# imazen/codec-eval

Hardware: AMD Instinct MI355X
Metric: metric MP/s (SSIMULACRA2+DSSIM+Butteraugli) at 1/2/4/8 GPU; HBM-roofline % (higher is better)
Workload: dtype f32

## Files before the change

codec-eval_amd/csrc/butteraugli.hip:

```cpp
#include <algorithm>
#include <cmath>
#include <cstdlib>
#include <type_traits>

#include "ce_internal.h"

namespace {

constexpr int TPB = 256;
constexpr int PSY = 10;
enum { UHF0 = 0, UHF1, HF0, HF1, MF0, MF1, MF2, LF0, LF1, LF2 };

struct geom {
    uint32_t w, h, pitch;
    size_t plane;
};

struct blur_kernel {
    int len;
    float k[40];
    float lo[16], hi[16];
};

#define BA_XY                                                           \
// ... 370 lines not shown
    constexpr int NF = (RAW * (IW / 4) + TPB - 1) / TPB;
    float4 pf[NF];
    auto fetch = [&](int q) {
        const float *p = tmp + (EPI == EPI_MASK ? (size_t)slot : (size_t)slot * 3 + q) * g.plane;
#pragma unroll
        for (int m = 0; m < NF; m++) {
            const int i = m * TPB + (int)threadIdx.x, r = i / (IW / 4), X = x0 - (HV ? LEFT : 0) + 4 * (i % (IW / 4)), Y = y0 - off + r;
            float4 v = make_float4(0.f, 0.f, 0.f, 0.f);
            if (r < RAW && Y >= 0 && Y < (int)g.h && X >= 0 && X < (int)g.pitch) v = *reinterpret_cast<const float4 *>(p + (size_t)Y * g.pitch + X);
            v.x = X < (int)g.w ? v.x : 0.0f;
            v.y = X + 1 < (int)g.w ? v.y : 0.0f;
            v.z = X + 2 < (int)g.w ? v.z : 0.0f;
            v.w = X + 3 < (int)g.w ? v.w : 0.0f;
            pf[m] = v;
        }
    };
    auto stash = [&]() {
#pragma unroll
        for (int m = 0; m < NF; m++) {
            const int i = m * TPB + (int)threadIdx.x;
            if (i < RAW * (IW / 4)) *reinterpret_cast<float4 *>((HV ? in_t : tile) + 4 * i) = pf[m];
        }
    };
    constexpr int S0 = LEFT - off, NW = (S0 + 3 + LEN + 3) / 4;
    const int rc4 = 4 * ((int)threadIdx.x % (TW / 4));
    __shared__ __attribute__((aligned(16))) float s_sx[HV ? TW : 4];
    if (HV && threadIdx.x < TW)
        s_sx[threadIdx.x] = x0 + (int)threadIdx.x < (int)g.w ? border_scale<LEN>(bk, x0 + (int)threadIdx.x, (int)g.w, inv_wsum) : 0.0f;
    float scale_x[4] = {0.0f, 0.0f, 0.0f, 0.0f};
    fetch(0);
    if (HV) {
        stash();
        __syncthreads();
#pragma unroll
        for (int k = 0; k < 4; k++) scale_x[k] = s_sx[rc4 + k];
    }
#pragma unroll
    for (int q = 0; q < NP; q++) {
        if (HV) {
#pragma unroll 1
            for (int u = threadIdx.x; u < RAW * (TW / 4); u += TPB) {
                const int r = u / (TW / 4);
                const float4 *src = reinterpret_cast<const float4 *>(in_t + r * IW + rc4);
                float wnd[4 * NW];
#pragma unroll
                for (int m = 0; m < NW; m++) {
                    const float4 v = src[m];
                    wnd[4 * m] = v.x, wnd[4 * m + 1] = v.y, wnd[4 * m + 2] = v.z, wnd[4 * m + 3] = v.w;
                }
                float out[4];
#pragma unroll
                for (int k = 0; k < 4; k++) {
                    float sum = 0.0f;
#pragma unroll
                    for (int j = 0; j < LEN; j++) sum = blur_tap(sum, wnd[S0 + k + j], bk.k[j]);
                    out[k] = sum * scale_x[k];
                }
                *reinterpret_cast<float4 *>(tile + r * TW + rc4) = make_float4(out[0], out[1], out[2], out[3]);
            }
            __syncthreads();
            if (q + 1 < NP) fetch(q + 1);
        } else {
            if (q) __syncthreads();
            stash();
            if (q + 1 < NP) fetch(q + 1);
            __syncthreads();
        }
#pragma unroll
        for (int part = 0; part < PARTS; part++) {
            const int ly = 32 * part + 8 * wv, gy0 = y0 + ly;
            if (col_live && gy0 < (int)g.h) {
                float v[BW_OUT + LEN - 1];
#pragma unroll
                for (int j = 0; j < BW_OUT + LEN - 1; j++) v[j] = tile[(ly + j) * TW + c];
#pragma unroll
                for (int o = 0; o < BW_OUT; o++) {
                    float sum = 0.0f;
#pragma unroll
                    for (int j = 0; j < LEN; j++) sum = blur_tap(sum, v[o + j], bk.k[j]);
                    res[q][part][o] = sum * border_scale<LEN>(bk, gy0 + o, (int)g.h, inv_wsum);
                }
            }
        }
        if (HV && q + 1 < NP) {
            stash();
            __syncthreads();
        }
    }
    if (!col_live) return;
    const size_t pl = g.plane;
#pragma unroll
    for (int part = 0; part < PARTS; part++) {
        const int gy0 = y0 + 32 * part + 8 * wv;
        if (gy0 >= (int)g.h) break;
        float *ps = psy + (size_t)slot * PSY * g.plane + (size_t)gy0 * g.pitch + gx;
#pragma unroll
        for (int o = 0; o < BW_OUT; o++) {
            if (gy0 + o >= (int)g.h) break;
            float *q = ps + (size_t)o * g.pitch;
            const size_t ao = (size_t)slot * 3 * pl + (size_t)(gy0 + o) * g.pitch + gx;
            if (EPI == EPI_LF) {
                const float *xs = xyb + (size_t)slot * 3 * pl + (size_t)(gy0 + o) * g.pitch + gx;
                const float lx = res[0][part][o], ly = res[1][part][o], lb = res[2][part][o];
                aux_out[ao] = xs[0] - lx;
                aux_out[ao + pl] = xs[pl] - ly;
                aux_out[ao + 2 * pl] = xs[2 * pl] - lb;
                const float xmul = 33.832837186260f, ymul = 14.458268100570f, bmul = 49.87984651440f, y_to_b_mul = -0.362267051518f;
                const float bb = __builtin_fmaf(y_to_b_mul, ly, lb);
                q[LF2 * pl] = bb * bmul;
                q[LF0 * pl] = lx * xmul;
                q[LF1 * pl] = ly * ymul;
            } else if (EPI == EPI_MF) {
                const float kRemoveMfRange = 0.29f, kAddMfRange = 0.1f;
                const float mf0 = res[0][part][o], mf1 = res[1][part][o];
                const float hf0 = tmp[ao] - mf0, hf1 = tmp[ao + pl] - mf1;
                q[MF0 * pl] = remove_range(kRemoveMfRange, mf0);
                q[MF1 * pl] = amplify_range(kAddMfRange, mf1);
                q[MF2 * pl] = res[2][part][o];
                const float suppress = 46.0f, sv = 0.653020556257f, one_minus_s = 1.0f - 0.653020556257f;
                const float scaler = __builtin_fmaf(suppress / __builtin_fmaf(hf1, hf1, suppress), one_minus_s, sv);
                aux_out[ao] = scaler * hf0;
                aux_out[ao + pl] = hf1;
            } else if (EPI == EPI_MASK) {
                aux_out[(size_t)slot * pl + (size_t)(gy0 + o) * g.pitch + gx] = res[0][part][o];
            } else {
                const float kRemoveHfRange = 1.5f, kAddHfRange = 0.132f, kRemoveUhfRange = 0.04f;
                const float kMaxclampHf = 28.4691806922f, kMaxclampUhf = 5.19175294647f, kMulYHf = 2.155f, kMulYUhf = 2.69313763794f;
                float hf0_out, uhf0_out, hf1_out, uhf1_out;
                {
                    const float hf = res[0][part][o];
                    const float uhf = tmp[ao] - hf;
                    hf0_out = remove_range(kRemoveHfRange, hf);
                    uhf0_out = remove_range(kRemoveUhfRange, uhf);
                    q[HF0 * pl] = hf0_out;
                    q[UHF0 * pl] = uhf0_out;
                }
                {
                    float hf = maximum_clamp(res[1][part][o], kMaxclampHf);
                    float uhf = tmp[ao + pl] - hf;
                    uhf = maximum_clamp(uhf, kMaxclampUhf);
                    uhf *= kMulYUhf;
                    uhf1_out = uhf;
                    q[UHF1 * pl] = uhf;
                    hf *= kMulYHf;
                    hf1_out = amplify_range(kAddHfRange, hf);
                    q[HF1 * pl] = hf1_out;
                }
                mask_in[(size_t)slot * pl + (size_t)(gy0 + o) * g.pitch + gx] = mask_pre_one(uhf0_out, hf0_out, uhf1_out, hf1_out);
            }
        }
    }
}

struct malta_params {
    float norm2_0gt1, norm2_0lt1, norm1;
};

struct mline {
    int n;
    signed char d[9][2];
};

__device__ constexpr mline MALTA_HF[16] = {
    {9, {{-4, 0}, {-3, 0}, {-2, 0}, {-1, 0}, {0, 0}, {1, 0}, {2, 0}, {3, 0}, {4, 0}}},
    {9, {{0, -4}, {0, -3}, {0, -2}, {0, -1}, {0, 0}, {0, 1}, {0, 2}, {0, 3}, {0, 4}}},
    {7, {{-3, -3}, {-2, -2}, {-1, -1}, {0, 0}, {1, 1}, {2, 2}, {3, 3}}},
    {7, {{3, -3}, {2, -2}, {1, -1}, {0, 0}, {-1, 1}, {-2, 2}, {-3, 3}}},
    {9, {{1, -4}, {1, -3}, {1, -2}, {0, -1}, {0, 0}, {0, 1}, {-1, 2}, {-1, 3}, {-1, 4}}},
    {9, {{-1, -4}, {-1, -3}, {-1, -2}, {0, -1}, {0, 0}, {0, 1}, {1, 2}, {1, 3}, {1, 4}}},
    {9, {{-4, -1}, {-3, -1}, {-2, -1}, {-1, 0}, {0, 0}, {1, 0}, {2, 1}, {3, 1}, {4, 1}}},
    {9, {{-4, 1}, {-3, 1}, {-2, 1}, {-1, 0}, {0, 0}, {1, 0}, {2, -1}, {3, -1}, {4, -1}}},
    {7, {{-2, -3}, {-1, -2}, {-1, -1}, {0, 0}, {1, 1}, {1, 2}, {2, 3}}},
    {7, {{2, -3}, {1, -2}, {1, -1}, {0, 0}, {-1, 1}, {-1, 2}, {-2, 3}}},
    {7, {{-3, -2}, {-2, -1}, {-1, -1}, {0, 0}, {1, 1}, {2, 1}, {3, 2}}},
    {7, {{3, -2}, {2, -1}, {1, -1}, {0, 0}, {-1, 1}, {-2, 1}, {-3, 2}}},
    {8, {{-4, 2}, {-3, 2}, {-2, 1}, {-1, 1}, {0, 0}, {1, 0}, {2, -1}, {3, -1}}},
    {8, {{-4, -2}, {-3, -2}, {-2, -1}, {-1, -1}, {0, 0}, {1, 0}, {2, 1}, {3, 1}}},
    {8, {{-2, -4}, {-2, -3}, {-1, -2}, {-1, -1}, {0, 0}, {0, 1}, {1, 2}, {1, 3}}},
    {8, {{2, -4}, {2, -3}, {1, -2}, {1, -1}, {0, 0}, {0, 1}, {-1, 2}, {-1, 3}}},
};
__device__ constexpr mline MALTA_LF[16] = {
    {5, {{-4, 0}, {-2, 0}, {0, 0}, {2, 0}, {4, 0}}},
    {5, {{0, -4}, {0, -2}, {0, 0}, {0, 2}, {0, 4}}},
    {5, {{-3, -3}, {-2, -2}, {0, 0}, {2, 2}, {3, 3}}},
    {5, {{3, -3}, {2, -2}, {0, 0}, {-2, 2}, {-3, 3}}},
    {5, {{1, -4}, {1, -2}, {0, 0}, {-1, 2}, {-1, 4}}},
    {5, {{-1, -4}, {-1, -2}, {0, 0}, {1, 2}, {1, 4}}},
    {5, {{-4, -1}, {-2, -1}, {0, 0}, {2, 1}, {4, 1}}},
    {5, {{-4, 1}, {-2, 1}, {0, 0}, {2, -1}, {4, -1}}},
    {5, {{-2, -3}, {-1, -2}, {0, 0}, {1, 2}, {2, 3}}},
    {5, {{2, -3}, {1, -2}, {0, 0}, {-1, 2}, {-2, 3}}},
    {5, {{-3, -2}, {-2, -1}, {0, 0}, {2, 1}, {3, 2}}},
    {5, {{3, -2}, {2, -1}, {0, 0}, {-2, 1}, {-3, 2}}},
    {5, {{-4, 2}, {-2, 1}, {0, 0}, {2, -1}, {4, -2}}},
    {5, {{-4, -2}, {-2, -1}, {0, 0}, {2, 1}, {4, 2}}},
    {5, {{-2, -4}, {-1, -2}, {0, 0}, {1, 2}, {2, 4}}},
    {5, {{2, -4}, {1, -2}, {0, 0}, {-1, 2}, {-2, 4}}},
};

constexpr int MT = 64, MH = 4, ML = MT + 2 * MH;

__device__ constexpr bool malta_line_descends(const mline &ln)
{
    for (int j = 1; j < ln.n; j++)
        if (ln.d[j][1] > ln.d[j - 1][1]) return false;
    return ln.d[0][1] != ln.d[ln.n - 1][1];
}
__device__ constexpr bool malta_line_monotone(const mline &ln)
{
    bool up = true, down = true;
    for (int j = 1; j < ln.n; j++) {
        if (ln.d[j][1] < ln.d[j - 1][1]) up = false;
        if (ln.d[j][1] > ln.d[j - 1][1]) down = false;
    }
    return up || down;
}
__device__ constexpr bool malta_tables_monotone()
{
    for (int k = 0; k < 16; k++)
        if (!malta_line_monotone(MALTA_HF[k]) || !malta_line_monotone(MALTA_LF[k])) return false;
    return true;
}
static_assert(malta_tables_monotone(), "the row-streaming Malta unit needs every line's rows to be visited in one direction");

struct malta_bands {
    malta_params p[2][3];
};

__device__ __forceinline__ void div2_shared_rcp(float a0, float a1, float b, float &q0, float &q1)
{
    const float r = ce_rcp_refined(b);
    q0 = ce_div_refined(a0, b, r);
    q1 = ce_div_refined(a1, b, r);
}

__device__ __forceinline__ float malta_pre_diff(float v0, float v1, const malta_params &mp)
{
    const float absval = 0.5f * (fabsf(v0) + fabsf(v1));
    const float diff = v0 - v1;
    float scaler, scaler2;
    div2_shared_rcp(mp.norm2_0gt1, mp.norm2_0lt1, mp.norm1 + absval, scaler, scaler2);
    const float r = scaler * diff;
    const float fabs0 = fabsf(v0), too_small = 0.55f * fabs0, too_big = 1.05f * fabs0;
    const bool neg = v0 < 0;
    const float u = neg ? -v1 : v1;
    const bool lo = u < too_small, hi = u > too_big;
    const float impact = scaler2 * (lo ? too_small - u : u - too_big);
    const float rn = r + ((neg == lo) ? -impact : impact);
    return (lo || hi) ? rn : r;
}

__device__ __forceinline__ float l2_asym_acc(float total, float val0, float val1, float vw_0gt1, float vw_0lt1)
{
    const float diff = val0 - val1;
    total = __builtin_fmaf(diff * diff, vw_0gt1, total);
    const float fabs0 = fabsf(val0);
    const float too_small = 0.4f * fabs0, too_big = fabs0;
    const float if_neg = val1 > -too_small ? val1 + too_small : (val1 < -too_big ? -val1 - too_big : 0.0f);
    const float if_pos = val1 < too_small ? too_small - val1 : (val1 > too_big ? val1 - too_big : 0.0f);
    const float v = val0 < 0.0f ? if_neg : if_pos;
    return __builtin_fmaf(vw_0lt1, v * v, total);
}

template <bool LF>
__device__ __forceinline__ void malta_rows_xy(const ba_f2 *__restrict__ base, ba_f2 (&acc)[2])
{
    ba_f2 sum[2][16];
    ba_f2 parked[2][16][9];
#pragma unroll
    for (int r = 0; r < 9; r++) {
        ba_f2 v[10];
        const float4 *row = reinterpret_cast<const float4 *>(base + r * ML);
#pragma unroll
        for (int q = 0; q < 5; q++) {
            const float4 t = row[q];
            v[2 * q] = ba_f2{t.x, t.y};
            v[2 * q + 1] = ba_f2{t.z, t.w};
        }
        const int dy = r - 4;
#pragma unroll
        for (int o = 0; o < 2; o++) {
#pragma unroll
            for (int k = 0; k < 16; k++) {
                const mline &ln = LF ? MALTA_LF[k] : MALTA_HF[k];
                if (!malta_line_descends(ln)) {
#pragma unroll
                    for (int j = 0; j < 9; j++)
                        if (j < ln.n && ln.d[j][1] == dy) {
                            const ba_f2 t = v[4 + o + ln.d[j][0]];
                            sum[o][k] = j == 0 ? t : sum[o][k] + t;
                        }
                } else if (dy == ln.d[0][1]) {
                    ba_f2 acc_k = {0.0f, 0.0f};
#pragma unroll
                    for (int j = 0; j < 9; j++)
                        if (j < ln.n) {
                            const ba_f2 t = ln.d[j][1] == dy ? v[4 + o + ln.d[j][0]] : parked[o][k][j];
                            acc_k = j == 0 ? t : acc_k + t;
                        }
                    sum[o][k] = acc_k;
                } else {
#pragma unroll
                    for (int j = 0; j < 9; j++)
                        if (j < ln.n && ln.d[j][1] == dy) parked[o][k][j] = v[4 + o + ln.d[j][0]];
                }
            }
// ... 366 lines not shown
        b->ba_psy[l] = b->ba_diff[l] = b->ba_mask[l] = nullptr;
    }
    for (auto &p : b->ba_s) hipFree(p), p = nullptr;
    for (auto &p : b->ba_s_half) hipFree(p), p = nullptr;
    if (b->ba_half_stream) hipStreamSynchronize(b->ba_half_stream);
    if (b->ev_ba_fork) hipEventDestroy(b->ev_ba_fork);
    if (b->ev_ba_join) hipEventDestroy(b->ev_ba_join);
    b->ba_half_stream = nullptr;
    b->ev_ba_fork = b->ev_ba_join = nullptr;
    hipFree(b->ba_blk_max);
    hipFree(b->ba_blk_sums);
    hipFree(b->ba_pnorm);
    hipFree(b->ba_map);
    hipFree(b->ba_cells);
    b->ba_map = b->ba_cells = nullptr;
    b->ba_cells_cap = 0;
    b->ba_map_pairs = 0;
    b->ba_blk_max = nullptr;
    b->ba_blk_sums = nullptr;
    b->ba_pnorm = nullptr;
    b->ba_ref_src = nullptr;
    b->ba_ready = false;
}

static int ba_allocate(ce_batch *b)
{
    ce_ctx *ctx = b->ctx;
    auto set = [](ce_batch::ba_level &d, uint32_t w, uint32_t h) {
        d.w = w;
        d.h = h;
        d.pitch = (w + 31u) & ~31u;
        d.plane = (size_t)d.pitch * h;
    };
    set(b->ba[0], b->w, b->h);
    set(b->ba[1], (b->w + 1) / 2, (b->h + 1) / 2);
    b->ba_levels = (b->ba[1].w >= 8 && b->ba[1].h >= 8) ? 2 : 1;
    const size_t slots = (size_t)b->max_refs + b->max_pairs, P = b->max_pairs, p0 = b->ba[0].plane;
    for (int l = 0; l < b->ba_levels; l++) {
        CE_HIP(ctx, hipMalloc(&b->ba_psy[l], slots * PSY * b->ba[l].plane * sizeof(float)));
        if (l == 1) CE_HIP(ctx, hipMalloc(&b->ba_diff[l], P * b->ba[l].plane * sizeof(float)));
    }
    for (auto &p : b->ba_s) CE_HIP(ctx, hipMalloc(&p, slots * 3 * p0 * sizeof(float)));
    for (int l = 0; l < b->ba_levels; l++) {
        CE_HIP(ctx, hipMalloc(&b->ba_mask[l], slots * b->ba[l].plane * sizeof(float)));
        CE_HIP(ctx, hipMalloc(&b->ba_mask_vals[l], (size_t)b->max_refs * 2 * b->ba[l].plane * sizeof(float)));
    }
    b->ba_blocks = ((b->ba[0].w + 63) / 64) * ((b->ba[0].h + 3) / 4);
    CE_HIP(ctx, hipMalloc(&b->ba_blk_max, P * b->ba_blocks * sizeof(float)));
    CE_HIP(ctx, hipMalloc(&b->ba_blk_sums, P * b->ba_blocks * 3 * sizeof(double)));
    CE_HIP(ctx, hipMalloc(&b->ba_pnorm, P * sizeof(double)));
    return CE_OK;
}

static int ba_prepare(ce_batch *b)
{
    if (b->ba_ready) return CE_OK;
    const int rc = ba_allocate(b);
    if (rc != CE_OK) {
        const std::string why = b->ctx->err;
        ce_butteraugli_free(b);
        (void)hipGetLastError();
        b->ctx->err = why;
        return rc;
    }
    b->ba_ready = true;
    return CE_OK;
}

int ce_launch_butteraugli(ce_batch *b, const uint8_t *d_refs, uint32_t n_refs_used, uint32_t n_pairs, float intensity_target,
                          bool store_map)
{
    ce_ctx *ctx = b->ctx;
    int rc = ba_prepare(b);
    if (rc != CE_OK) return rc;
    if (store_map && !b->ba_map && hipMalloc(&b->ba_map, (size_t)b->max_pairs * b->ba[0].plane * sizeof(float)) != hipSuccess) {
        b->ba_map = nullptr;
        (void)hipGetLastError();
        ctx->err = "out of device memory for the Butteraugli diffmaps";
        return CE_ERR_BACKEND;
    }
    const uint32_t n_slots = n_refs_used + n_pairs, mr = b->max_refs;
    const bool cached = b->keep_ref_pyramid && b->ba_ref_src == d_refs && b->ba_ref_count >= n_refs_used && b->ba_ref_intensity == intensity_target;
    const uint32_t z0 = cached ? n_refs_used : 0, nz = n_slots - z0;
    if (!cached) b->ref_builds[2]++;
    const blur_kernel k12 = make_kernel(1.2f), kLf = make_kernel(7.15593339443f), kHf = make_kernel(3.22489901262f),
                      kUhf = make_kernel(1.56416327805f), kMask = make_kernel(2.7f);
    float sw = 0.0f;
    for (int j = 0; j < 5; j++) sw += k12.k[j];
    const float sc = 1.0f / sw, w0 = k12.k[2] * sc, w1 = k12.k[3] * sc, w2 = k12.k[4] * sc;
    const double hf_asymmetry = 1.0;
    const malta_params mUhfY = make_malta(1.10039032555 * hf_asymmetry, 1.10039032555 / hf_asymmetry, 71.7800275169, false);
    const malta_params mUhfX = make_malta(173.5 * hf_asymmetry, 173.5 / hf_asymmetry, 5.0, false);
    const malta_params mHfY = make_malta(18.7237414387 * std::sqrt(hf_asymmetry), 18.7237414387 / std::sqrt(hf_asymmetry), 4498534.45232, true);
    const malta_params mHfX = make_malta(6923.99476109 * std::sqrt(hf_asymmetry), 6923.99476109 / std::sqrt(hf_asymmetry), 8051.15833247, true);
    const malta_params mMfY = make_malta(37.0819870399, 37.0819870399, 130262059.556, true);
    const malta_params mMfX = make_malta(8246.75321353, 8246.75321353, 1009002.70582, true);

    const bool two_streams = b->ba_levels == 2 && !ctx->prof_serial && (double)n_pairs * b->w * b->h <= 4e6;
    hipStream_t s_main = CE_STREAM(ctx), s_half = s_main;
    if (two_streams) {
        if (!b->ba_half_stream) {
            if (!(b->ba_half_stream = ce_ctx_aux_stream(ctx, ce_ctx::AUX_BA_HALF))) return CE_ERR_BACKEND;
            CE_HIP(ctx, hipEventCreateWithFlags(&b->ev_ba_fork, hipEventDisableTiming));
            CE_HIP(ctx, hipEventCreateWithFlags(&b->ev_ba_join, hipEventDisableTiming));
            const size_t slots = (size_t)b->max_refs + b->max_pairs;
            for (auto &p : b->ba_s_half) CE_HIP(ctx, hipMalloc(&p, slots * 3 * b->ba[1].plane * sizeof(float)));
        }
        s_half = b->ba_half_stream;
        CE_HIP(ctx, hipEventRecord(b->ev_ba_fork, s_main));
        CE_HIP(ctx, hipStreamWaitEvent(s_half, b->ev_ba_fork, 0));
    }
    uint32_t final_tiles = 0;
    for (int l = b->ba_levels - 1; l >= 0; l--) {
        const auto &d = b->ba[l];
        const geom g{d.w, d.h, d.pitch, d.plane};
        const dim3 gx((d.w + 63) / 64, (d.h + 3) / 4, 1);
        auto G = [&](uint32_t z) { return dim3(gx.x, gx.y, z); };
        hipStream_t st = l == 1 ? s_half : s_main;
        float *const *scr = (two_streams && l == 1) ? b->ba_s_half : b->ba_s;
        float *psy = b->ba_psy[l], *sA = scr[0], *sC = scr[2];
        const plane_sel s3{3, 0, 3};
        const dim3 ft((d.w + FT - 1) / FT, (d.h + FT - 1) / FT, nz);
        if (l == 0) {
            CE_LAUNCH_ON(ctx, st, "ba_front_u8", k_ba_front<false>, ft, dim3(TPB), 0, d_refs, b->d_tests, ctx->d_lut_ssim2, g, sC, g, w0, w1, w2,
                      intensity_target, b->img_bytes, n_refs_used, mr, z0);
        } else {
            const auto &pd = b->ba[0];
            CE_LAUNCH_ON(ctx, st, "ba_front_half", k_ba_front<true>, ft, dim3(TPB), 0, d_refs, b->d_tests, ctx->d_lut_ssim2,
                      geom{pd.w, pd.h, pd.pitch, pd.plane}, sC, g, w0, w1, w2, intensity_target, b->img_bytes, n_refs_used, mr, z0);
        }
        {
            if (kLf.len != 33 || kHf.len != 15 || kUhf.len != 7) {
                ctx->err = "unexpected blur kernel length";
                return CE_ERR_BACKEND;
            }
            const dim3 gh3((g.w + 255) / 256, (g.h + 8 * BH_TILES - 1) / (8 * BH_TILES), nz * 3);
            float *sB = scr[1];
            CE_LAUNCH_ON(ctx, st, "ba_blur_h33", k_ba_blur_h<33>, gh3, dim3(TPB), 0, (const float *)sC, sA, g, s3, s3, kLf, inv_weight_sum(kLf),
                      n_refs_used, mr, 1, z0);
            const dim3 gvs((g.w + 63) / 64, (g.h + 31) / 32, nz);
            CE_LAUNCH_ON(ctx, st, "ba_blur_v_lf", (k_ba_blur_v_split<33, EPI_LF, false, 32>), gvs, dim3(TPB), 0, (const float *)sA,
                         (const float *)sC, psy, g, kLf, inv_weight_sum(kLf), n_refs_used, mr, z0, (float *)nullptr, sB);
            CE_LAUNCH_ON(ctx, st, "ba_blur_hv_mf", (k_ba_blur_v_split<15, EPI_MF, true, 32>), gvs, dim3(TPB), 0, (const float *)sB,
                         (const float *)nullptr, psy, g, kHf, inv_weight_sum(kHf), n_refs_used, mr, z0, (float *)nullptr, sA);
            CE_LAUNCH_ON(ctx, st, "ba_blur_hv_hf", (k_ba_blur_v_split<7, EPI_HF, true, 32>), gvs, dim3(TPB), 0, (const float *)sA,
                         (const float *)nullptr, psy, g, kUhf, inv_weight_sum(kUhf), n_refs_used, mr, z0, sB, (float *)nullptr);
        }

        {
            if (kMask.len != 13) {
                ctx->err = "unexpected blur kernel length";
                return CE_ERR_BACKEND;
            }
            const dim3 gm((g.w + 63) / 64, (g.h + 31) / 32, nz);
            CE_LAUNCH_ON(ctx, st, "ba_blur_hv_mask", (k_ba_blur_v_split<13, EPI_MASK, true, 32>), gm, dim3(TPB), 0, (const float *)scr[1],
                      (const float *)nullptr, psy, g, kMask, inv_weight_sum(kMask), n_refs_used, mr, z0, (float *)nullptr, b->ba_mask[l]);
        }
        if (!cached)
            CE_LAUNCH_ON(ctx, st, "ba_mask_vals", k_ba_mask_vals, G(n_refs_used), dim3(TPB), 0, (const float *)b->ba_mask[l], b->ba_mask_vals[l], g);

        malta_bands mb;
        mb.p[0][0] = mUhfX; mb.p[0][1] = mHfX; mb.p[0][2] = mMfX;
        mb.p[1][0] = mUhfY; mb.p[1][1] = mHfY; mb.p[1][2] = mMfY;
        const uint32_t tiles_x = (d.w + MT - 1) / MT, tiles_y = (d.h + 31) / 32;
        if ((rc = ce_build_xcd_list(b, n_pairs, ce_xcd_keys{1, tiles_x * tiles_y, 1}, &b->ba_work[l])) != CE_OK) return rc;
        const bool has_sub = b->ba_levels == 2;
        const auto &ds = b->ba[has_sub ? 1 : 0];
        const geom gsub{ds.w, ds.h, ds.pitch, ds.plane};
#define CE_MALTA_ARGS(FINAL, STORE)                                                                                                \
    psy, b->d_pair_ref, (const float *)b->ba_mask[l], (const float *)b->ba_mask_vals[l],                                               \
        STORE ? b->ba_map : FINAL ? (float *)nullptr : b->ba_diff[1], g, mr, mb, (const uint2 *)b->ba_work[l].d, tiles_x,             \
        FINAL ? (const float *)b->ba_diff[1] : (const float *)nullptr, gsub, has_sub ? 1 : 0, b->ba_blk_max, b->ba_blk_sums, b->ba_blocks
        const dim3 gmalta(b->ba_work[l].len);
        if (l == 0) {
            final_tiles = tiles_x * tiles_y;
            if (two_streams) CE_HIP(ctx, hipStreamWaitEvent(s_main, b->ev_ba_join, 0));
            if (store_map)
                CE_LAUNCH_ON(ctx, st, "ba_malta_l2_map", (k_ba_malta_l2_xy<32, 256, true, true>), gmalta, dim3(256), 0, CE_MALTA_ARGS(true, true));
            else
                CE_LAUNCH_ON(ctx, st, "ba_malta_l2", (k_ba_malta_l2_xy<32, 256, true, false>), gmalta, dim3(256), 0, CE_MALTA_ARGS(true, false));
        } else {
            CE_LAUNCH_ON(ctx, st, "ba_malta_l2", (k_ba_malta_l2_xy<32, 256, false, false>), gmalta, dim3(256), 0, CE_MALTA_ARGS(false, false));
            if (two_streams) CE_HIP(ctx, hipEventRecord(b->ev_ba_join, s_half));
        }
#undef CE_MALTA_ARGS
    }
    if (b->keep_ref_pyramid && !cached) {
        b->ba_ref_src = d_refs;
        b->ba_ref_count = n_refs_used;
        b->ba_ref_intensity = intensity_target;
    }
    const auto &d0 = b->ba[0];
    CE_LAUNCH(ctx, "ba_score", k_ba_score, dim3(n_pairs), dim3(TPB), 0, b->ba_blk_max, b->ba_blk_sums, b->d_scores, b->ba_pnorm,
              b->ba_blocks, final_tiles, (double)d0.w * (double)d0.h);
    CE_HIP(ctx, hipGetLastError());
    return CE_OK;
}

int ce_butteraugli_read_maps(ce_batch *b, uint32_t first, uint32_t count, uint32_t block, float *out)
{
    ce_ctx *ctx = b->ctx;
    const auto &d = b->ba[0];
    const geom g{d.w, d.h, d.pitch, d.plane};
    if (block == 1) {
        CE_HIP(ctx, hipMemcpy2DAsync(out, (size_t)d.w * sizeof(float), b->ba_map + (size_t)first * d.plane, (size_t)d.pitch * sizeof(float),
                                     (size_t)d.w * sizeof(float), (size_t)count * d.h, hipMemcpyDeviceToHost, ctx->stream));
        CE_HIP(ctx, hipStreamSynchronize(ctx->stream));
        return CE_OK;
    }
    uint32_t lb = 0;
    while ((1u << lb) < block) lb++;
    const uint32_t bw = (d.w + block - 1) >> lb, bh = (d.h + block - 1) >> lb, tiles_x = (d.w + 255) / 256;
    const size_t n = (size_t)count * bw * bh;
    if (b->ba_cells_cap < n) {
        hipFree(b->ba_cells);
        b->ba_cells = nullptr;
        b->ba_cells_cap = 0;
        CE_HIP(ctx, hipMalloc(&b->ba_cells, n * sizeof(float)));
        b->ba_cells_cap = n;
    }
    const size_t blocks = (size_t)tiles_x * bh * count;
    if (blocks > 0x7fffffffu) {
        ctx->err = "diffmap readout too large for one launch";
        return CE_ERR_INVALID_ARG;
    }
    CE_LAUNCH_ON(ctx, ctx->stream, "ba_block_max", k_ba_block_max, dim3((uint32_t)blocks), dim3(256), 0, (const float *)b->ba_map, g, first,
                 lb, tiles_x, bw, bh, b->ba_cells);
    CE_HIP(ctx, hipGetLastError());
    CE_HIP(ctx, hipMemcpyAsync(out, b->ba_cells, n * sizeof(float), hipMemcpyDeviceToHost, ctx->stream));
    CE_HIP(ctx, hipStreamSynchronize(ctx->stream));
    return CE_OK;
}
```

profiles/make_traffic.py:

```python
#!/usr/bin/env python3
import collections
import csv
import glob
import importlib
import json
import os
import re
import sys

HERE = os.path.dirname(os.path.abspath(__file__))
sys.path.insert(0, os.path.dirname(HERE))

SHORT = [
    (r"k_ssim2_hblur_lds<-1>", "ssim2_hblur_L1-5"), (r"k_ssim2_vblur_dma<-1>", "ssim2_vblur_ssim_L1-5"),
    (r"k_ssim2_hblur_lds<0>", "ssim2_hblur_L0"), (r"k_ssim2_vblur_dma<0>", "ssim2_vblur_ssim_L0"),
    (r"k_ssim2_prep<true>", "ssim2_prep_u8"), (r"k_ssim2_prep<false>", "ssim2_prep"), (r"k_ssim2_finalize", "ssim2_finalize"),
    (r"k_dssim_create_stream<true", "dssim_create_u8"), (r"k_dssim_create_stream<false", "dssim_create"), (r"k_dssim_create<true>", "dssim_create_u8"), (r"k_dssim_create<false>", "dssim_create"), (r"k_dssim_compare", "dssim_compare"),
    (r"k_dssim_avg", "dssim_avg"), (r"k_dssim_absdev", "dssim_absdev"), (r"k_dssim_finalize_pairs", "dssim_finalize"),
    (r"k_ba_front<false>", "ba_front_u8"), (r"k_ba_front<true>", "ba_front_half"), (r"k_ba_subsample2x_u8", "ba_subsample2x"),
    (r"k_ba_blur_h<(\d+)>", "ba_blur_h{}"), (r"k_ba_blur_v<(\d+)>", "ba_blur_v{}"),
    (r"k_ba_blur_v_split<13", "ba_blur_hv_mask"), (r"k_ba_blur_v_split<33", "ba_blur_v_lf"), (r"k_ba_blur_v_split<15, *1, *true", "ba_blur_hv_mf"), (r"k_ba_blur_v_split<7, *2, *true", "ba_blur_hv_hf"),
    (r"k_ba_blur_v_split<15", "ba_blur_v_mf"), (r"k_ba_blur_v_split<7", "ba_blur_v_hf"),
    (r"k_ba_malta_l2_xy", "ba_malta_l2"), (r"k_ba_mask_pre", "ba_mask_pre"), (r"k_ba_mask_vals", "ba_mask_vals"), (r"k_ba_mask_combine", "ba_mask_combine"),
    (r"k_ba_final", "ba_final"), (r"k_ba_score", "ba_score"), (r"k_psnr_sse", "psnr_sse"), (r"k_psnr_clear", "psnr_clear"),
    (r"k_xyb_roundtrip", "xyb_roundtrip"), (r"k_calib_read<(\d+)>", "calib_read_b{}"), (r"k_calib_write<(\d+)>", "calib_write_b{}"),
]
READ_WIDTH_16 = ("ssim2_hblur", "ssim2_vblur", "ba_blur_h", "ba_blur_v_", "ba_malta_l2")
READ_WIDTH_1 = ("dssim_create_u8", "ba_subsample2x")
WRITE_WIDTH_16 = ("ssim2_hblur", "ba_blur_h")


def short(name):
    for pat, fmt in SHORT:
        m = re.search(pat, name)
        if m:
            return fmt.format(*m.groups())
    return name.split("(")[0][-48:]


def one(d, suffix):
    f = glob.glob(os.path.join(d, "**", "*" + suffix), recursive=True)
    if not f:
        raise SystemExit(f"no *{suffix} under {d}")
    return max(f, key=os.path.getmtime)


def counters_of(d, cname):
    acc, n = collections.defaultdict(float), collections.Counter()
    for r in csv.DictReader(open(one(d, "counter_collection.csv"))):
        if r["Counter_Name"] != cname:
            continue
        k = short(r["Kernel_Name"])
        acc[k] += float(r["Counter_Value"])
        n[k] += 1
    return {k: acc[k] / n[k] for k in acc}, dict(n)


def main():
    if sys.argv[1] == "--stats-only":
        tag, fetch_dir, write_dir, sidecar = None, None, None, None
        stats_dir, stats_tag = sys.argv[2], sys.argv[3]
    else:
        tag, fetch_dir, write_dir, sidecar = sys.argv[1:5]
        stats_dir = sys.argv[5] if len(sys.argv) > 5 else None
        stats_tag = sys.argv[6] if len(sys.argv) > 6 else tag
    if stats_dir:
        rows = list(csv.DictReader(open(one(stats_dir, "kernel_stats.csv"))))
        with open(os.path.join(HERE, f"{stats_tag}_kernel_stats.csv"), "w", newline="") as fo:
            w = csv.writer(fo)
            w.writerow(["Kernel", "Calls", "TotalDurationNs", "AverageNs", "Percentage", "MinNs", "MaxNs"])
            groups = collections.OrderedDict()
            for r in rows:
                groups.setdefault(short(r["Name"]), []).append(r)
            for name, rs in groups.items():
                if len(rs) == 1:
                    r = rs[0]
                    w.writerow([name, r["Calls"], r["TotalDurationNs"], r["AverageNs"], r["Percentage"], r["MinNs"], r["MaxNs"]])
                    continue
                calls = sum(int(r["Calls"]) for r in rs)
                total = sum(int(r["TotalDurationNs"]) for r in rs)
                w.writerow([name, calls, total, f"{total / calls:.6f}", f"{sum(float(r['Percentage']) for r in rs):.2f}",
                            min(int(r["MinNs"]) for r in rs), max(int(r["MaxNs"]) for r in rs)])
                for r in rs:
                    inst = re.search(r"<([^>]*)>", r["Name"])
                    w.writerow([f"{name} [instance <{inst.group(1) if inst else '?'}>]", r["Calls"], r["TotalDurationNs"], r["AverageNs"],
                                r["Percentage"], r["MinNs"], r["MaxNs"]])
    if sidecar is None:
        return
    side = json.load(open(sidecar))
    rf = importlib.import_module("codec-eval_amd.roofline")
    alg = rf.step_bytes([rf.Bucket(side["width"], side["height"], side["n_refs"], side["n_pairs"])], side["metrics"], side["xyb_roundtrip"])
    px0 = side["n_pairs"] * side["width"] * side["height"]
    fetch, n_f = counters_of(fetch_dir, "FETCH_SIZE")
    write, n_w = counters_of(write_dir, "WRITE_SIZE")
    cal = side["calib_bytes"]
    f_read = {w_: cal / (fetch[f"calib_read_b{w_}"] * 1024) for w_ in (1, 4, 16) if fetch.get(f"calib_read_b{w_}")}
    f_write = {w_: cal / (write[f"calib_write_b{w_}"] * 1024) for w_ in (4, 16) if write.get(f"calib_write_b{w_}")}
    out = {
        "_provenance": "rocprofv3 --kernel-trace --pmc FETCH_SIZE / --pmc WRITE_SIZE, two separate passes over "
                       f"profiles/prof_step.py {side['config']} {side['steps']}; counters are KiB, averaged per launch; corrected by the "
                       "per-width factors MEASURED in the same passes from the calibration streams (bytes moved / bytes reported); "
                       "produced by profiles/make_traffic.py",
        "_launch": dict(side, scale0_pixels=px0),
        "_calibration": {"read_factor_by_lane_bytes": {str(k): round(v, 4) for k, v in f_read.items()},
                         "write_factor_by_lane_bytes": {str(k): round(v, 4) for k, v in f_write.items()}},
    }
    with open(os.path.join(HERE, f"{tag}_pmc_fetch_write.csv"), "w", newline="") as fo:
        w = csv.writer(fo)
        w.writerow(["Kernel", "launches_per_step", "FETCH_SIZE_KiB_per_launch", "WRITE_SIZE_KiB_per_launch"])
        for k in sorted(set(fetch) | set(write)):
            f, wr = fetch.get(k, 0.0), write.get(k, 0.0)
            lps = n_f.get(k, n_w.get(k, 0)) / (1 if k.startswith("calib_") else side["steps"])
            w.writerow([k, round(lps, 2), round(f, 1), round(wr, 1)])
            if k.startswith(("calib_", "__amd")):
                continue
            rw = 16 if k.startswith(READ_WIDTH_16) else 1 if k.startswith(READ_WIDTH_1) else 4
            ww = 16 if k.startswith(WRITE_WIDTH_16) else 4
            fb = f * 1024 * f_read.get(rw, 1.0)
            wb = wr * 1024 * f_write.get(ww, 1.0)
            per_step = (fb + wb) * lps
            out[k] = {"launches_per_step": round(lps, 2), "fetch_bytes_per_launch": fb, "write_bytes_per_launch": wb,
                      "hbm_bytes_per_launch": fb + wb, "hbm_bytes_per_step": per_step, "bytes_per_scale0_pixel": round(per_step / px0, 2),
                      "read_lane_bytes": rw, "write_lane_bytes": ww}
            if k in alg:
                out[k]["algorithmic_bytes_per_step"] = alg[k]
                out[k]["algorithmic_bytes_per_scale0_pixel"] = round(alg[k] / px0, 2)
                out[k]["traffic_over_algorithmic"] = round(per_step / alg[k], 3)
    json.dump(out, open(os.path.join(HERE, f"traffic_{tag}.json"), "w"), indent=1)
    print("calibration", out["_calibration"])
    for k, v in out.items():
        if not k.startswith("_"):
            print(f"{k:24s} {v['bytes_per_scale0_pixel']:8.2f} B/px0   alg {v.get('algorithmic_bytes_per_scale0_pixel', float('nan')):8.2f}")


if __name__ == "__main__":
    main()
```

Measured before the change: 19040.

## Replace mask blur with single-wave vertical strip kernel using register sliding window

Adds a new separable blur kernel for the mask stage. Each 64-thread block walks down a 64-column strip: it prefetches rows into registers, runs the horizontal pass through LDS, and keeps the vertical window in registers, so halo rows are not re-read per tile. Strip height is picked adaptively to keep enough waves in flight. The trade-off is more serial work per block and fewer threads per block, which can hurt occupancy and latency hiding on small images.

```diff
diff --git a/codec-eval_amd/csrc/butteraugli.hip b/codec-eval_amd/csrc/butteraugli.hip
--- a/codec-eval_amd/csrc/butteraugli.hip
+++ b/codec-eval_amd/csrc/butteraugli.hip
@@ -546,6 +546,103 @@
     }
 }
 
+template <int LEN>
+__global__ __launch_bounds__(64) void k_ba_blur_hv_strip(const float *__restrict__ in, float *__restrict__ out, geom g, blur_kernel bk,
+                                                         float inv_wsum, uint32_t n_refs_used, uint32_t max_refs, uint32_t z0, uint32_t sh)
+{
+    constexpr int off = LEN / 2, TW = 64, SR = 8, LEFT = 8, IW = TW + 2 * LEFT;
+    static_assert(off <= LEFT, "row-pass halo");
+    constexpr int P = (LEN - 1 + SR - 1) / SR, PAD = P * SR - (LEN - 1), WN = (P + 1) * SR;
+    __shared__ __attribute__((aligned(16))) float in_t[SR * IW];
+    __shared__ __attribute__((aligned(16))) float rb[SR * TW];
+    __shared__ __attribute__((aligned(16))) float s_sx[TW];
+    const uint32_t slot = slot_of(blockIdx.z + z0, n_refs_used, max_refs);
+    const float *p = in + (size_t)slot * g.plane;
+    const int x0 = blockIdx.x * TW, ys = blockIdx.y * (int)sh, ye = min(ys + (int)sh, (int)g.h);
+    const int t = threadIdx.x, gx = x0 + t;
+    const int y_in = ys - off - PAD, steps = P + (ye - ys + SR - 1) / SR;
+    constexpr int NF = (SR * (IW / 4) + 63) / 64;
+    float4 pf[NF];
+    auto fetch = [&](int y) {
+#pragma unroll
+        for (int m = 0; m < NF; m++) {
+            const int i = m * 64 + t, r = i / (IW / 4), X = x0 - LEFT + 4 * (i % (IW / 4)), Y = y + r;
+            float4 v = make_float4(0.f, 0.f, 0.f, 0.f);
+            if (r < SR && Y >= 0 && Y < (int)g.h && X >= 0 && X < (int)g.pitch) v = *reinterpret_cast<const float4 *>(p + (size_t)Y * g.pitch + X);
+            v.x = X < (int)g.w ? v.x : 0.0f;
+            v.y = X + 1 < (int)g.w ? v.y : 0.0f;
+            v.z = X + 2 < (int)g.w ? v.z : 0.0f;
+            v.w = X + 3 < (int)g.w ? v.w : 0.0f;
+            pf[m] = v;
+        }
+    };
+    constexpr int S0 = LEFT - off, NW = (S0 + 3 + LEN + 3) / 4;
+    const int rc4 = 4 * (t % (TW / 4)), rr = t / (TW / 4);
+    s_sx[t] = gx < (int)g.w ? border_scale<LEN>(bk, gx, (int)g.w, inv_wsum) : 0.0f;
+    fetch(y_in);
+    __syncthreads();
+    float scale_x[4];
+#pragma unroll
+    for (int k = 0; k < 4; k++) scale_x[k] = s_sx[rc4 + k];
+    float win[WN];
+#pragma unroll
+    for (int j = 0; j < WN; j++) win[j] = 0.0f;
+#pragma unroll 1
+    for (int s = 0; s < steps; s++) {
+#pragma unroll
+        for (int m = 0; m < NF; m++) {
+            const int i = m * 64 + t;
+            if (i < SR * (IW / 4)) *reinterpret_cast<float4 *>(in_t + 4 * i) = pf[m];
+        }
+        if (s + 1 < steps) fetch(y_in + SR * (s + 1));
+        __syncthreads();
+#pragma unroll
+        for (int h2 = 0; h2 < SR / 4; h2++) {
+            const int r = rr + 4 * h2;
+            const float4 *src = reinterpret_cast<const float4 *>(in_t + r * IW + rc4);
+            float wnd[4 * NW];
+#pragma unroll
+            for (int m = 0; m < NW; m++) {
+                const float4 v = src[m];
+                wnd[4 * m] = v.x, wnd[4 * m + 1] = v.y, wnd[4 * m + 2] = v.z, wnd[4 * m + 3] = v.w;
+            }
+            float o4[4];
+#pragma unroll
+            for (int k = 0; k < 4; k++) {
+                float sum = 0.0f;
+#pragma unroll
+                for (int j = 0; j < LEN; j++) sum = blur_tap(sum, wnd[S0 + k + j], bk.k[j]);
+                o4[k] = sum * scale_x[k];
+            }
+            *reinterpret_cast<float4 *>(rb + r * TW + rc4) = make_float4(o4[0], o4[1], o4[2], o4[3]);
+        }
+        __syncthreads();
+#pragma unroll
+        for (int j = 0; j < WN - SR; j++) win[j] = win[j + SR];
+#pragma unroll
+        for (int r = 0; r < SR; r++) win[WN - SR + r] = rb[r * TW + t];
+        if (s < P || gx >= (int)g.w) continue;
+        const int y0 = ys + SR * (s - P);
+#pragma unroll
+        for (int o = 0; o < SR; o++) {
+            if (y0 + o >= ye) break;
+            float sum = 0.0f;
+#pragma unroll
+            for (int j = 0; j < LEN; j++) sum = blur_tap(sum, win[PAD + o + j], bk.k[j]);
+            out[(size_t)slot * g.plane + (size_t)(y0 + o) * g.pitch + gx] = sum * border_scale<LEN>(bk, y0 + o, (int)g.h, inv_wsum);
+        }
+    }
+}
+
+uint32_t ba_strip_rows(uint32_t strips, uint32_t h, uint32_t n_images)
+{
+    auto waves = [&](uint32_t rows) { return (size_t)strips * ((h + rows - 1) / rows) * n_images; };
+    uint32_t rows = 128;
+    while (rows > 32 && waves(rows) < 8192) rows /= 2;
+    while (rows > 8 && waves(rows) < 2048) rows /= 2;
+    return rows;
+}
+
 struct malta_params {
     float norm2_0gt1, norm2_0lt1, norm1;
 };
@@ -1218,9 +1315,9 @@
                 ctx->err = "unexpected blur kernel length";
                 return CE_ERR_BACKEND;
             }
-            const dim3 gm((g.w + 63) / 64, (g.h + 31) / 32, nz);
-            CE_LAUNCH_ON(ctx, st, "ba_blur_hv_mask", (k_ba_blur_v_split<13, EPI_MASK, true, 32>), gm, dim3(TPB), 0, (const float *)scr[1],
-                      (const float *)nullptr, psy, g, kMask, inv_weight_sum(kMask), n_refs_used, mr, z0, (float *)nullptr, b->ba_mask[l]);
+            const uint32_t strips = (g.w + 63) / 64, sh = ba_strip_rows(strips, g.h, nz);
+            CE_LAUNCH_ON(ctx, st, "ba_blur_hv_mask", k_ba_blur_hv_strip<13>, dim3(strips, (g.h + sh - 1) / sh, nz), dim3(64), 0,
+                         (const float *)scr[1], b->ba_mask[l], g, kMask, inv_weight_sum(kMask), n_refs_used, mr, z0, sh);
         }
         if (!cached)
             CE_LAUNCH_ON(ctx, st, "ba_mask_vals", k_ba_mask_vals, G(n_refs_used), dim3(TPB), 0, (const float *)b->ba_mask[l], b->ba_mask_vals[l], g);
diff --git a/profiles/make_traffic.py b/profiles/make_traffic.py
--- a/profiles/make_traffic.py
+++ b/profiles/make_traffic.py
@@ -19,7 +19,7 @@
     (r"k_dssim_avg", "dssim_avg"), (r"k_dssim_absdev", "dssim_absdev"), (r"k_dssim_finalize_pairs", "dssim_finalize"),
     (r"k_ba_front<false>", "ba_front_u8"), (r"k_ba_front<true>", "ba_front_half"), (r"k_ba_subsample2x_u8", "ba_subsample2x"),
     (r"k_ba_blur_h<(\d+)>", "ba_blur_h{}"), (r"k_ba_blur_v<(\d+)>", "ba_blur_v{}"),
-    (r"k_ba_blur_v_split<13", "ba_blur_hv_mask"), (r"k_ba_blur_v_split<33", "ba_blur_v_lf"), (r"k_ba_blur_v_split<15, *1, *true", "ba_blur_hv_mf"), (r"k_ba_blur_v_split<7, *2, *true", "ba_blur_hv_hf"),
+    (r"k_ba_blur_hv_strip<13", "ba_blur_hv_mask"), (r"k_ba_blur_v_split<13", "ba_blur_hv_mask"), (r"k_ba_blur_v_split<33", "ba_blur_v_lf"), (r"k_ba_blur_v_split<15, *1, *true", "ba_blur_hv_mf"), (r"k_ba_blur_v_split<7, *2, *true", "ba_blur_hv_hf"),
     (r"k_ba_blur_v_split<15", "ba_blur_v_mf"), (r"k_ba_blur_v_split<7", "ba_blur_v_hf"),
     (r"k_ba_malta_l2_xy", "ba_malta_l2"), (r"k_ba_mask_pre", "ba_mask_pre"), (r"k_ba_mask_vals", "ba_mask_vals"), (r"k_ba_mask_combine", "ba_mask_combine"),
     (r"k_ba_final", "ba_final"), (r"k_ba_score", "ba_score"), (r"k_psnr_sse", "psnr_sse"), (r"k_psnr_clear", "psnr_clear"),
```

After: 19070 (median of 4 runs). Within noise of the previous version (+0.2%).
